# google/uis-rnn

Measured on NVIDIA H100. Metric: predict_frames_per_sec_beam10_256d, higher is better.
Workload: dtype f32

## Files before the change

### uisrnn_b200/csrc/uis_beam.cuh

```cuda
#pragma once
#include "uis_common.cuh"
#include "uis_beam_tc.cuh"
#include "uis_beam_stat.cuh"

namespace uis {

constexpr int kStages = 2;
constexpr int kStageBytes = 48 * 1024;
constexpr int kInitSlot = 0;
#ifndef UIS_CP_BEAM
#define UIS_CP_BEAM 20
#endif
constexpr int kCPBeam = UIS_CP_BEAM;
template <int H> struct BeamCP { static constexpr int value = H > 512 ? 8 : kCPBeam; };
template <int H> __host__ __device__ constexpr int beam_cp() { return BeamCP<H>::value; }
constexpr int kCPCluster = 12;
constexpr int kXchVals = 24;
constexpr int kCPTree = 16;
template <int H> struct TreeCP { static constexpr int value = H > 512 ? 8 : kCPTree; };
template <int H> __host__ __device__ constexpr int tree_cp() { return TreeCP<H>::value; }
constexpr int kMaxLanes = 8;
constexpr int kMaxBeam = 128;
constexpr int kMaxDepth = 4;

// ... 375 lines not shown
  const uint32_t base = smem_u32(mine + tid);
  float sum[NV];
#pragma unroll
  for (int i = 0; i < NV; ++i) sum[i] = 0.f;
  for (unsigned r = 0; r < x.size; ++r) {
    if (r == x.rank) {
#pragma unroll
      for (int i = 0; i < NV; ++i) sum[i] = (r == 0) ? v[i] : __fadd_rn(sum[i], v[i]);
    } else {
      const uint32_t ra = dsmem_addr(base, r);
      float4 t[NV / 4];
#pragma unroll
      for (int i = 0; i < NV / 4; ++i) t[i] = dsmem_ld_f32x4(ra + (uint32_t)(i * NT) * 16u);
#pragma unroll
      for (int i = 0; i < NV / 4; ++i) {
        sum[4 * i + 0] = (r == 0) ? t[i].x : __fadd_rn(sum[4 * i + 0], t[i].x);
        sum[4 * i + 1] = (r == 0) ? t[i].y : __fadd_rn(sum[4 * i + 1], t[i].y);
        sum[4 * i + 2] = (r == 0) ? t[i].z : __fadd_rn(sum[4 * i + 2], t[i].z);
        sum[4 * i + 3] = (r == 0) ? t[i].w : __fadd_rn(sum[4 * i + 3], t[i].w);
      }
    }
  }
#pragma unroll
  for (int i = 0; i < NV; ++i) v[i] = sum[i];
  x.count += 1;
}
template <int NT>
__device__ __forceinline__ void xch_barrier(XchCtx& x, int tid) {
  const unsigned b = x.count & 1u, parity = (x.count >> 1) & 1u;
  named_bar_sync(1, NT);
  if (tid == 0)
    for (unsigned r = 0; r < x.size; ++r)
      if (r != x.rank) mbar_arrive_remote(dsmem_addr(smem_u32(&x.bar[b]), r));
  mbar_wait_cluster(&x.bar[b], parity);
  x.count += 1;
}

struct ColCtx {
  const int* lane;
  const int* src;
  const int* dst;
  const int* vis;
  const long long* girow;
};

template <class C, int NC, bool DEEP, bool XCL = false>
__device__ __forceinline__ void run_pass(const BeamParams& p, const float* ring, uint64_t* full, uint64_t* empty,
                                         unsigned& it, float* XA, float* XB,
                                         const ColCtx cc, int m0, int Mp, float* pool_mean_cta,
                                         float* pool_hidden_cta, const float (&bh)[C::RG], const float (&b1r)[C::UPT],
                                         float b2r, int tid, int lane, long long* ph, long long& tmark,
                                         XchCtx* xc = nullptr) {
  const int xrank = XCL ? (int)xc->rank : 0, xsize = XCL ? (int)xc->size : 1;
  constexpr int H = C::H, D = C::D, NT = C::NT, UPT = C::UPT;
  const int DH = p.depth * H;
  const size_t lane_pool_h = (size_t)p.P * DH, lane_pool_m = (size_t)p.P * D;
  {
    float acc[C::RG][4 * NC];
    lin_pass<C, 3 * H, C::KT_HH, 1, C::RG, NC, true, XCL>(ring, full, empty, it, XA, acc, tid, lane, xrank, xsize);
    if constexpr (XCL) {
      static_assert(!DEEP && 4 * C::RG <= kXchVals, "cluster mode: depth 1");
#pragma unroll
      for (int c = 0; c < NC; ++c) {
        float v[4 * C::RG];
#pragma unroll
        for (int i = 0; i < C::RG; ++i)
#pragma unroll
          for (int q = 0; q < 4; ++q) v[4 * i + q] = acc[i][4 * c + q];
        xch_allreduce<NT, 4 * C::RG>(*xc, v, tid);
#pragma unroll
        for (int i = 0; i < C::RG; ++i)
#pragma unroll
          for (int q = 0; q < 4; ++q) acc[i][4 * c + q] = v[4 * i + q];
      }
    }
#pragma unroll
    for (int u = 0; u < UPT; ++u) {
      const int j = tid + NT * u;
#pragma unroll
      for (int c = 0; c < NC; ++c) {
        const float4 hold = reinterpret_cast<const float4*>(XA + (size_t)j * C::CP)[c];
        const float ho[4] = {hold.x, hold.y, hold.z, hold.w};
        float hn[4];
#pragma unroll
        for (int q = 0; q < 4; ++q) {
          const int m = 4 * c + q;
          hn[q] = 0.f;
          if (m < Mp) {
            const float* gi = p.gi + (size_t)cc.girow[m0 + m] * 3 * H;
            const float r = sigmoid_f32(__fadd_rn(gi[j], __fadd_rn(acc[0 * UPT + u][m], bh[0 * UPT + u])));
            const float z = sigmoid_f32(__fadd_rn(gi[H + j], __fadd_rn(acc[1 * UPT + u][m], bh[1 * UPT + u])));
            const float n = tanhf(__fadd_rn(gi[2 * H + j], __fmul_rn(r, __fadd_rn(acc[2 * UPT + u][m], bh[2 * UPT + u]))));
            hn[q] = __fadd_rn(__fmul_rn(__fsub_rn(ho[q], n), z), n);
            pool_hidden_cta[(size_t)cc.lane[m0 + m] * lane_pool_h + (size_t)cc.dst[m0 + m] * DH + j] = hn[q];
          }
        }
        reinterpret_cast<float4*>(XB + (size_t)j * C::CP)[c] = make_float4(hn[0], hn[1], hn[2], hn[3]);
      }
    }
  }
  if constexpr (DEEP)
  for (int l = 1; l < p.depth; ++l) {
    named_bar_sync(1, NT);
    float acc[C::RG][4 * NC];
    lin_pass<C, 3 * H, C::KT_HH, 1, C::RG, NC>(ring, full, empty, it, XB, acc, tid, lane);
    float ni[UPT][4 * NC];
#pragma unroll
    for (int u = 0; u < UPT; ++u)
#pragma unroll
      for (int m = 0; m < 4 * NC; ++m) { ni[u][m] = acc[2 * UPT + u][m]; acc[2 * UPT + u][m] = 0.f; }
    named_bar_sync(1, NT);
#pragma unroll
    for (int u = 0; u < UPT; ++u) {
      const int j = tid + NT * u;
#pragma unroll
      for (int c = 0; c < NC; ++c) {
        float hv[4];
#pragma unroll
        for (int q = 0; q < 4; ++q) {
          const int m = 4 * c + q;
          hv[q] = (m < Mp) ? pool_hidden_cta[(size_t)cc.lane[m0 + m] * lane_pool_h + (size_t)cc.src[m0 + m] * DH +
                                             (size_t)l * H + j]
                           : 0.f;
        }
        reinterpret_cast<float4*>(XA + (size_t)j * C::CP)[c] = make_float4(hv[0], hv[1], hv[2], hv[3]);
      }
    }
    named_bar_sync(1, NT);
    lin_pass<C, 3 * H, C::KT_HH, 1, C::RG, NC, false>(ring, full, empty, it, XA, acc, tid, lane);
    const float* bi = p.bih_up + (size_t)(l - 1) * 3 * H;
    const float* bhl = p.bhh_up + (size_t)(l - 1) * 3 * H;
    float hn_out[UPT][4 * NC];
#pragma unroll
    for (int u = 0; u < UPT; ++u) {
      const int j = tid + NT * u;
      const float bir = bi[j], biz = bi[H + j], bin = bi[2 * H + j];
      const float bhr = bhl[j], bhz = bhl[H + j], bhn = bhl[2 * H + j];
#pragma unroll
      for (int c = 0; c < NC; ++c) {
        const float4 hold = reinterpret_cast<const float4*>(XA + (size_t)j * C::CP)[c];
        const float ho[4] = {hold.x, hold.y, hold.z, hold.w};
#pragma unroll
        for (int q = 0; q < 4; ++q) {
          const int m = 4 * c + q;
          const float r = sigmoid_f32(__fadd_rn(__fadd_rn(acc[0 * UPT + u][m], bir), bhr));
          const float z = sigmoid_f32(__fadd_rn(__fadd_rn(acc[1 * UPT + u][m], biz), bhz));
          const float n = tanhf(__fadd_rn(__fadd_rn(ni[u][m], bin), __fmul_rn(r, __fadd_rn(acc[2 * UPT + u][m], bhn))));
          const float hnew = __fadd_rn(__fmul_rn(__fsub_rn(ho[q], n), z), n);
          hn_out[u][m] = (m < Mp) ? hnew : 0.f;
          if (m < Mp)
            pool_hidden_cta[(size_t)cc.lane[m0 + m] * lane_pool_h + (size_t)cc.dst[m0 + m] * DH + (size_t)l * H + j] = hnew;
        }
      }
    }
    named_bar_sync(1, NT);
#pragma unroll
    for (int u = 0; u < UPT; ++u)
#pragma unroll
      for (int c = 0; c < NC; ++c)
        reinterpret_cast<float4*>(XB + (size_t)(tid + NT * u) * C::CP)[c] =
            make_float4(hn_out[u][4 * c], hn_out[u][4 * c + 1], hn_out[u][4 * c + 2], hn_out[u][4 * c + 3]);
  }
  named_bar_sync(1, NT);
  if (tid == 0) { const long long now_ = clock64(); ph[2] += now_ - tmark; tmark = now_; }
  {
    float acc[C::R1][4 * NC];
    lin_pass<C, H, C::KT_1, C::KG1, C::R1, NC, true, XCL>(ring, full, empty, it, XB, acc, tid, lane, xrank, xsize);
    float out[UPT][4 * NC];
    ksplit_reduce<C, H, C::KG1, C::R1, UPT, NC>(acc, XA, out, tid);
    if constexpr (XCL) {
      static_assert(UPT * 4 * NC <= kXchVals, "cluster mode: W1 exchange in one round");
      float v[UPT * 4 * NC];
#pragma unroll
      for (int u = 0; u < UPT; ++u)
#pragma unroll
        for (int m = 0; m < 4 * NC; ++m) v[u * 4 * NC + m] = out[u][m];
      xch_allreduce<NT, UPT * 4 * NC>(*xc, v, tid);
#pragma unroll
      for (int u = 0; u < UPT; ++u)
#pragma unroll
        for (int m = 0; m < 4 * NC; ++m) out[u][m] = v[u * 4 * NC + m];
    }
#pragma unroll
    for (int u = 0; u < UPT; ++u)
#pragma unroll
      for (int c = 0; c < NC; ++c) {
        float4 v;
        v.x = fmaxf(__fadd_rn(out[u][4 * c + 0], b1r[u]), 0.f); v.y = fmaxf(__fadd_rn(out[u][4 * c + 1], b1r[u]), 0.f);
        v.z = fmaxf(__fadd_rn(out[u][4 * c + 2], b1r[u]), 0.f); v.w = fmaxf(__fadd_rn(out[u][4 * c + 3], b1r[u]), 0.f);
        reinterpret_cast<float4*>(XA + (size_t)(tid + NT * u) * C::CP)[c] = v;
      }
  }
  named_bar_sync(1, NT);
  if (tid == 0) { const long long now_ = clock64(); ph[3] += now_ - tmark; tmark = now_; }
  {
    float mu_old[4 * NC];
#pragma unroll
    for (int m = 0; m < 4 * NC; ++m)
      mu_old[m] = (m < Mp && tid < D)
                      ? pool_mean_cta[(size_t)cc.lane[m0 + m] * lane_pool_m + (size_t)cc.src[m0 + m] * D + tid]
                      : 0.f;
    float acc[C::R2][4 * NC];
    lin_pass<C, D, C::KT_2, C::KG2, C::R2, NC, true, XCL>(ring, full, empty, it, XA, acc, tid, lane, xrank, xsize);
    float out[1][4 * NC];
    ksplit_reduce<C, D, C::KG2, C::R2, 1, NC>(acc, XA, out, tid);
    if constexpr (XCL) xch_allreduce<NT, 4 * NC>(*xc, out[0], tid);
    if (tid < D) {
#pragma unroll
      for (int m = 0; m < 4 * NC; ++m) {
        if (m < Mp) {
          const float mval = __fadd_rn(out[0][m], b2r);
          const int n = cc.vis[m0 + m];
          const float mu = (n == 0) ? mval
                                    : __fdiv_rn(__fadd_rn(__fmul_rn(mu_old[m], (float)(n - 1)), mval), (float)n);
          pool_mean_cta[(size_t)cc.lane[m0 + m] * lane_pool_m + (size_t)cc.dst[m0 + m] * D + tid] = mu;
        }
      }
    }
  }
}

template <class C, bool DEEP, bool XCL = false>
__device__ __forceinline__ void run_pass_any(const BeamParams& p, const float* ring, uint64_t* full, uint64_t* empty,
                                             unsigned& it, float* XA, float* XB, const ColCtx cc, int m0, int Mp,
                                             float* pool_mean_cta, float* pool_hidden_cta, const float (&bh)[C::RG],
                                             const float (&b1r)[C::UPT], float b2r, int tid, int lane, long long* ph,
                                             long long& tmark, XchCtx* xc = nullptr) {
  const int nc = (Mp + 3) / 4;
#define UIS_RP(NCV, DEEPV) \
  run_pass<C, NCV, DEEPV, XCL>(p, ring, full, empty, it, XA, XB, cc, m0, Mp, pool_mean_cta, pool_hidden_cta, bh, b1r, b2r, tid, lane, ph, tmark, xc)
  if (nc == 1) UIS_RP(1, DEEP); else if (nc == 2) UIS_RP(2, DEEP); else if (nc == 3 || C::CP < 16) UIS_RP(3, DEEP);
  else if (nc == 4 || C::CP < 20) { if constexpr (C::CP >= 16) UIS_RP(4, DEEP); }
  else { if constexpr (C::CP >= 20) UIS_RP(5, DEEP); }
#undef UIS_RP
}

template <int H, int D, int CP, int NT>
__device__ __forceinline__ void stat_pass(const BeamParams& p, const float* sW, float* XA, float* XB, const ColCtx cc, int m0,
                                          int Mp, float* pool_mean_g, float* pool_hidden_g, float* scratch_g, unsigned* bar,
                                          unsigned& epoch, int q, int tid, long long* ph, long long& tmark) {
  using S = StatCfg<H, D>;
  const size_t lane_pool_h = (size_t)p.P * H, lane_pool_m = (size_t)p.P * D;
  stat_dot<H, S::R0, CP, NT>(sW, S::LD, 0, XA, XB, Mp, tid);
  named_bar_sync(1, NT);
  if (tid < S::UG * CP) {
    const int m = tid % CP, u = tid / CP, j = q * S::UG + u;
    if (m < Mp) {
      const float ar = stat_sum<S::R0, CP, NT>(XB, 0 * S::UG + u, m);
      const float az = stat_sum<S::R0, CP, NT>(XB, 1 * S::UG + u, m);
      const float an = stat_sum<S::R0, CP, NT>(XB, 2 * S::UG + u, m);
      const float* gi = p.gi + (size_t)cc.girow[m0 + m] * 3 * H;
      const float r = sigmoid_f32(__fadd_rn(gi[j], __fadd_rn(ar, __ldg(p.bhh + j))));
      const float z = sigmoid_f32(__fadd_rn(gi[H + j], __fadd_rn(az, __ldg(p.bhh + H + j))));
      const float n = tanhf(__fadd_rn(gi[2 * H + j], __fmul_rn(r, __fadd_rn(an, __ldg(p.bhh + 2 * H + j)))));
      const float ho = XA[(size_t)j * CP + m];
      pool_hidden_g[(size_t)cc.lane[m0 + m] * lane_pool_h + (size_t)cc.dst[m0 + m] * H + j] =
          __fadd_rn(__fmul_rn(__fsub_rn(ho, n), z), n);
    }
  }
  stat_group_sync<NT>(bar, epoch, tid);
  if (tid == 0) { const long long now_ = clock64(); ph[2] += now_ - tmark; tmark = now_; }
  for (int i = tid; i < Mp * H; i += NT) {
    const int m = i / H, k = i % H;
    XA[(size_t)k * CP + m] = __ldcg(pool_hidden_g + (size_t)cc.lane[m0 + m] * lane_pool_h + (size_t)cc.dst[m0 + m] * H + k);
  }
  named_bar_sync(1, NT);
  stat_dot<H, S::R1, CP, NT>(sW, S::LD, S::R0, XA, XB, Mp, tid);
  named_bar_sync(1, NT);
  if (tid < S::R1 * CP) {
    const int m = tid % CP, u = tid / CP, j = q * S::R1 + u;
    if (m < Mp)
      scratch_g[(size_t)m * H + j] = fmaxf(__fadd_rn(stat_sum<S::R1, CP, NT>(XB, u, m), __ldg(p.b1 + j)), 0.f);
  }
  stat_group_sync<NT>(bar, epoch, tid);
  if (tid == 0) { const long long now_ = clock64(); ph[3] += now_ - tmark; tmark = now_; }
  for (int i = tid; i < Mp * H; i += NT) {
    const int m = i / H, k = i % H;
    XA[(size_t)k * CP + m] = __ldcg(scratch_g + (size_t)m * H + k);
  }
  named_bar_sync(1, NT);
  stat_dot<H, S::R2, CP, NT>(sW, S::LD, S::R0 + S::R1, XA, XB, Mp, tid);
  named_bar_sync(1, NT);
  if (tid < S::R2 * CP) {
    const int m = tid % CP, u = tid / CP, d = q * S::R2 + u;
    if (m < Mp) {
      const float mval = __fadd_rn(stat_sum<S::R2, CP, NT>(XB, u, m), __ldg(p.b2 + d));
      const int n = cc.vis[m0 + m];
      const float mu_old = __ldcg(pool_mean_g + (size_t)cc.lane[m0 + m] * lane_pool_m + (size_t)cc.src[m0 + m] * D + d);
      const float mu = (n == 0) ? mval : __fdiv_rn(__fadd_rn(__fmul_rn(mu_old, (float)(n - 1)), mval), (float)n);
      pool_mean_g[(size_t)cc.lane[m0 + m] * lane_pool_m + (size_t)cc.dst[m0 + m] * D + d] = mu;
    }
  }
  stat_group_sync<NT>(bar, epoch, tid);
}

template <int H, int D, int N, class Idle>
__device__ __forceinline__ void tc_run_pass(const BeamParams& p, const unsigned char* ring, unsigned char* bop,
                                            const TcBars& tb, unsigned& tbox, const ColCtx cc, int m0, int Mp,
                                            float* pool_mean_cta, float* pool_hidden_cta, float* scratch_cta, int tid,
                                            int lane, int warp, long long* ph, long long& tmark, long long* tstat,
                                            Idle idle_work) {
  using TC = TcCfg<H, D, N>;
  constexpr int NT = 256, NI = N / 8;
  constexpr int KB = (NI == 6) ? 2 : 4, WB = (NI == 6) ? 3 : NI;
  auto hslot = [&](int g, int s) { return pool_hidden_cta + (size_t)(g * p.P + s) * H; };
  auto mslot = [&](int g, int s) { return pool_mean_cta + (size_t)(g * p.P + s) * D; };
  const int wg = warp >> 2;
  const int r0 = wg * 64 + (warp & 3) * 16 + (lane >> 2);
  const int cq = 2 * (lane & 3);
  long long* ts = (tid == 0) ? tstat : nullptr;
  const long long t_in = clock64();
  float acc[TC::NACC];
  auto stage_b = [&](auto src, float scale) {
    const long long w0 = clock64();
    tc_gather_b<H, N, NT>(bop, src, Mp, scale, tid);
    tc_publish_b<NT>();
    if (ts) ts[2] += clock64() - w0;
  };
  if (tid < Mp && (tid == 0 || cc.lane[m0 + tid] != cc.lane[m0 + tid - 1]))
    prefetch_l2_bulk(p.gi + (size_t)cc.girow[m0 + tid] * 3 * H, 3 * H * 4);
  stage_b([&](int m) -> const float* {
    return hslot(cc.lane[m0 + m], cc.src[m0 + m]); }, p.tc_sh);
  if (tid == 0) { const long long now_ = clock64(); ph[1] += now_ - tmark; tmark = now_; }
  idle_work();
  if (tid == 0) { const long long now_ = clock64(); ph[7] += now_ - tmark; tmark = now_; }
  static_assert(H >= NT, "gate parking: 2 * (N / 2) * NT floats within the [N][H] scratch");
  float* park = scratch_cta + tid;
  for (int ut = 0; ut < TC::UT; ++ut) {
    const int j0 = ut * 128 + r0;
    {
      float v[TC::NV];
#pragma unroll
      for (int g = 0; g < 2; ++g) {
        tc_tile<TC>(acc, ring, bop, tb, tbox, wg, lane, ts);
        tc_fold<TC>(acc, v, p.tc_inv_hh);
        const float bh[2] = {__ldg(p.bhh + g * H + j0), __ldg(p.bhh + g * H + j0 + 8)};
#pragma unroll
        for (int q = 0; q < TC::NV; ++q) park[(g * TC::NV + q) * NT] = __fadd_rn(v[q], bh[(q >> 1) & 1]);
      }
    }
    tc_tile<TC>(acc, ring, bop, tb, tbox, wg, lane, ts);
    float an[TC::NV];
    tc_fold<TC>(acc, an, p.tc_inv_hh);
    {
      const float bh[2] = {__ldg(p.bhh + 2 * H + j0), __ldg(p.bhh + 2 * H + j0 + 8)};
#pragma unroll
      for (int q = 0; q < TC::NV; ++q) an[q] = __fadd_rn(an[q], bh[(q >> 1) & 1]);
    }
#pragma unroll
    for (int k0 = 0; k0 < 2 * NI; k0 += KB) {
      float gr[KB][2], gz[KB][2], gn[KB][2], pr[KB][2], pz[KB][2], ho[KB][2];
#pragma unroll
      for (int b = 0; b < KB; ++b) {
        const int i = (k0 + b) >> 1, e = (k0 + b) & 1, m = 8 * i + cq + e;
        if (m < Mp) {
          const float* gi = p.gi + (size_t)cc.girow[m0 + m] * 3 * H + j0;
          const float* hs = hslot(cc.lane[m0 + m], cc.src[m0 + m]) + j0;
#pragma unroll
          for (int h = 0; h < 2; ++h) {
            const int v = 4 * i + 2 * h + e;
            gr[b][h] = __ldg(gi + 8 * h); gz[b][h] = __ldg(gi + H + 8 * h); gn[b][h] = __ldg(gi + 2 * H + 8 * h);
            pr[b][h] = park[v * NT]; pz[b][h] = park[(TC::NV + v) * NT];
            ho[b][h] = hs[8 * h];
          }
        }
      }
#pragma unroll
      for (int b = 0; b < KB; ++b) {
        const int i = (k0 + b) >> 1, e = (k0 + b) & 1, m = 8 * i + cq + e;
        if (m < Mp) {
          float* hd = hslot(cc.lane[m0 + m], cc.dst[m0 + m]) + j0;
#pragma unroll
          for (int h = 0; h < 2; ++h) {
            const int v = 4 * i + 2 * h + e;
            const float rg = sigmoid_f32(__fadd_rn(gr[b][h], pr[b][h]));
            const float zg = sigmoid_f32(__fadd_rn(gz[b][h], pz[b][h]));
            const float ng = tanhf(__fadd_rn(gn[b][h], __fmul_rn(rg, an[v])));
            hd[8 * h] = __fadd_rn(__fmul_rn(__fsub_rn(ho[b][h], ng), zg), ng);
          }
        }
      }
    }
  }
  named_bar_sync(1, NT);
  if (tid == 0) { const long long now_ = clock64(); ph[2] += now_ - tmark; tmark = now_; }
  stage_b([&](int m) -> const float* {
    return hslot(cc.lane[m0 + m], cc.dst[m0 + m]); }, p.tc_sh);
  for (int mt = 0; mt < TC::T2; ++mt) {
    float v1[TC::NV];
    tc_tile<TC>(acc, ring, bop, tb, tbox, wg, lane, ts);
    tc_fold<TC>(acc, v1, p.tc_inv_1);
#pragma unroll
    for (int h = 0; h < 2; ++h) {
      const int j = mt * 128 + r0 + 8 * h;
      const float b1j = __ldg(p.b1 + j);
#pragma unroll
      for (int i = 0; i < NI; ++i)
#pragma unroll
        for (int e = 0; e < 2; ++e) {
          const int m = 8 * i + cq + e;
          if (m < Mp) scratch_cta[(size_t)m * H + j] = fmaxf(__fadd_rn(v1[4 * i + 2 * h + e], b1j), 0.f);
        }
    }
  }
  named_bar_sync(1, NT);
  if (tid == 0) { const long long now_ = clock64(); ph[3] += now_ - tmark; tmark = now_; }
  stage_b([&](int m) -> const float* { return scratch_cta + (size_t)m * H; }, p.tc_sa);
  for (int mt = 0; mt < TC::T3; ++mt) {
    float v2[TC::NV];
    tc_tile<TC>(acc, ring, bop, tb, tbox, wg, lane, ts);
    tc_fold<TC>(acc, v2, p.tc_inv_2);
#pragma unroll
    for (int h = 0; h < 2; ++h) {
      const int d = mt * 128 + r0 + 8 * h;
      const float b2d = __ldg(p.b2 + d);
#pragma unroll
      for (int i0 = 0; i0 < NI; i0 += WB) {
        float mu_old[WB][2];
#pragma unroll
        for (int b = 0; b < WB; ++b)
#pragma unroll
          for (int e = 0; e < 2; ++e) {
            const int m = 8 * (i0 + b) + cq + e;
            if (m < Mp) mu_old[b][e] = mslot(cc.lane[m0 + m], cc.src[m0 + m])[d];
          }
#pragma unroll
        for (int b = 0; b < WB; ++b)
#pragma unroll
          for (int e = 0; e < 2; ++e) {
            const int m = 8 * (i0 + b) + cq + e;
            if (m < Mp) {
              const float mval = __fadd_rn(v2[4 * (i0 + b) + 2 * h + e], b2d);
              const int n = cc.vis[m0 + m];
              const float mu = (n == 0) ? mval : __fdiv_rn(__fadd_rn(__fmul_rn(mu_old[b][e], (float)(n - 1)), mval), (float)n);
              mslot(cc.lane[m0 + m], cc.dst[m0 + m])[d] = mu;
            }
          }
      }
    }
  }
  if (ts) ts[3] += clock64() - t_in;
}

template <int H, int D, bool DEEP, int XM = 0, int TCN = 0>
__global__ void __launch_bounds__(Cfg<H, D>::BLOCK, 1) uis_beam_kernel(const __grid_constant__ BeamParams p) {
  constexpr bool XCL = XM == 1, STAT = XM == 2;
  using C = Cfg<H, D, (XCL || STAT) ? kCPCluster : BeamCP<H>::value>;
  constexpr int NT = C::NT, NW = C::NW, UPT = C::UPT;
  constexpr bool TC = TCN > 0;
  static_assert(!TC || (!DEEP && !XCL && !STAT && NT == 256 && C::REBALANCE), "tensor-core pass: depth 1, one CTA per lane group");
  static_assert(!STAT || (!DEEP && NT == 256), "stationary-weights mode: depth 1, 256 consumer threads");
  using TCC = TcCfg<TC ? H : 512, TC ? D : 256, TC ? TCN : 48>;
  extern __shared__ __align__(128) unsigned char smem_raw[];
  unsigned char* smem = TC ? reinterpret_cast<unsigned char*>((reinterpret_cast<uintptr_t>(smem_raw) + 1023) & ~(uintptr_t)1023)
                           : smem_raw;
  const int B = p.B, Kcap = p.Kcap, G = p.G;
  const SmemLayout L_ = make_layout<H, D, C::CP, XCL, TCN, STAT>(B, Kcap, G);
  const SmemLayout& L = TC ? p.tc_layout : L_;
  if constexpr (TC)
    if (p.tc_layout.total == 0) __trap();
  const int sq = STAT ? (int)(blockIdx.x % kStatGroup) : 0, sgroup = STAT ? (int)(blockIdx.x / kStatGroup) : 0;
  float* ring = reinterpret_cast<float*>(smem + L.ring);
  float* XA = reinterpret_cast<float*>(smem + L.xa);
  float* XB = reinterpret_cast<float*>(smem + L.xb);
  float* wv = reinterpret_cast<float*>(smem + L.wv);
  int* colarr = reinterpret_cast<int*>(smem + L.cols);
  uint64_t* full = reinterpret_cast<uint64_t*>(smem + L.bars);
  uint64_t* empty = full + (TC ? TCC::STAGES : kStages);
  volatile int* misc = reinterpret_cast<volatile int*>(smem + L.misc);
  TcBars tb{full, empty};

  const int tid = threadIdx.x, lane = tid & 31, warp = tid >> 5;

  if (tid == 0) {
    if constexpr (TC) {
      for (int s = 0; s < TCC::STAGES; ++s) {
        mbar_init(&tb.full[s], 1);
        mbar_init(&tb.empty[s], NW);
      }
    } else {
      for (int s = 0; s < kStages; ++s) {
        mbar_init(&full[s], 1);
        mbar_init(&empty[s], NW);
      }
    }
    for (int i = 0; i < 16; ++i) misc[i] = 0;
    if constexpr (TC)
      for (int i = 16; i < 20; ++i) reinterpret_cast<long long*>(smem + L.phase)[i] = 0;
    if constexpr (XCL) {
      uint64_t* xbar = reinterpret_cast<uint64_t*>(smem + L.xbar);
      mbar_init(&xbar[0], cluster_nctarank() - 1);
      mbar_init(&xbar[1], cluster_nctarank() - 1);
      misc[MI_QNEXT] = (int)cluster_id_x();
    }
    if constexpr (STAT) misc[MI_QNEXT] = sgroup;
    fence_mbar_init();
  }
  __syncthreads();
  if constexpr (XCL) cluster_sync_all();

  if (warp >= NW) {
    if constexpr (STAT) return;
    if constexpr (TC) asm volatile("setmaxnreg.dec.sync.aligned.u32 40;");
    else if constexpr (C::REBALANCE) asm volatile("setmaxnreg.dec.sync.aligned.u32 24;");
    if constexpr (TC) {
      if (warp == NW) tc_producer_loop<TCC, H>(&p.tc_wmap, reinterpret_cast<unsigned char*>(ring), tb, &misc[MI_DONE]);
    } else {
      if (warp == NW && lane == 0) producer_loop<C, XCL>(p, ring, full, empty, misc);
    }
    return;
  }
  if constexpr (TC) asm volatile("setmaxnreg.inc.sync.aligned.u32 232;");
  else if constexpr (C::REBALANCE && !STAT) asm volatile("setmaxnreg.inc.sync.aligned.u32 240;");

  auto lane_base = [&](int g) -> unsigned char* { return smem + L.lanes + (size_t)g * L.lane_stride; };
  auto LSp = [&](int g) -> volatile int* { return reinterpret_cast<volatile int*>(lane_base(g) + L.l_ls); };
  const int DH = p.depth * H;
  const size_t pool_m_stride = (size_t)p.P * D, pool_h_stride = (size_t)p.P * DH;
  float* pool_mean_cta = p.pool_mean + (size_t)(STAT ? sgroup : blockIdx.x) * G * pool_m_stride;
  float* pool_hidden_cta = p.pool_hidden + (size_t)(STAT ? sgroup : blockIdx.x) * G * pool_h_stride;
  unsigned* bp_cta = p.bp + (size_t)blockIdx.x * G * p.maxN * B;
  const unsigned PW = (unsigned)(p.P + 31) / 32;
  const float INF = __int_as_float(0x7f800000);
  const int bbits = B > 32 ? 7 : 5;

  float bh[C::RG], b1r[UPT];
#pragma unroll
  for (int i = 0; i < C::RG; ++i) bh[i] = TC ? 0.f : p.bhh[(i / UPT) * H + tid + NT * (i % UPT)];
#pragma unroll
  for (int u = 0; u < UPT; ++u) b1r[u] = TC ? 0.f : p.b1[tid + NT * u];
  const float b2r = (tid < D && !TC) ? p.b2[tid] : 0.f;
  unsigned tc_boxes = 0;
  float* tc_scratch_cta = TC ? p.tc_scratch + (size_t)blockIdx.x * (TC ? TCN : 1) * H : nullptr;
  if (tid < D) wv[tid] = p.wvec[tid];
  unsigned stat_epoch = 0;
  if constexpr (STAT) stat_load_weights<H, D, NT>(ring, p.whh_t, p.w1_t, p.w2_t, sq, tid);
  for (int g = 0; g < G; ++g) {
    if (tid < D) pool_mean_cta[g * pool_m_stride + (size_t)kInitSlot * D + tid] = p.mean0[tid];
    for (int q = tid; q < DH; q += NT) pool_hidden_cta[g * pool_h_stride + (size_t)kInitSlot * DH + q] = p.hidden0[q];
  }

  int* collane = colarr; int* colsrc = colarr + G * B; int* colnew = colarr + 2 * G * B;
  int* colvis = colarr + 3 * G * B;
  long long* colrow = reinterpret_cast<long long*>(colarr + 4 * G * B);
  const ColCtx cc{collane, colsrc, colnew, colvis, colrow};
  XchCtx xc{reinterpret_cast<float*>(smem + L.xch), reinterpret_cast<uint64_t*>(smem + L.xbar),
            XCL ? cluster_ctarank() : 0u, XCL ? cluster_nctarank() : 1u, 0u};
  const int xsize = (int)xc.size;
  const bool tap_leader = (!XCL || xc.rank == 0) && (!STAT || sq == 0);

  unsigned it = 0;
  long long* ph = reinterpret_cast<long long*>(smem + L.phase);
  if (tid == 0) {
    for (int i = 0; i < 16; ++i) ph[i] = 0;
    ph[10] = clock64();
  }
  long long& tmark = ph[10];
  long long& st_cols = ph[11]; long long& st_pass = ph[12]; long long& st_cand = ph[13]; long long& st_steps = ph[14];
  long long& st_maxk = ph[15];
#define UIS_PHASE(i)                         \
  do {                                       \
    if (tid == 0) {                          \
      const long long now_ = clock64();      \
      ph[i] += now_ - tmark;                 \
      tmark = now_;                          \
    }                                        \
  } while (0)

  auto lane_fetch = [&](int g) {
    volatile int* ls = LSp(g);
    for (;;) {
      int uidx;
      if constexpr (XCL) {
        uidx = misc[MI_QNEXT];
        misc[MI_QNEXT] = uidx + (int)cluster_nclusters_x();
      } else if constexpr (STAT) {
        uidx = misc[MI_QNEXT];
        misc[MI_QNEXT] = uidx + (int)(gridDim.x / kStatGroup);
      } else {
        uidx = atomicAdd(p.queue, 1);
      }
      if (uidx >= p.U) { ls[LS_ACTIVE] = 0; ls[LS_FRESH] = 0; return; }
      const int u = p.order[uidx];
      const long long row0 = p.row_off[u];
      const int N = (int)(p.row_off[u + 1] - row0);
      if (N == 0) {
        p.status[u] = 0;
        if (p.spk_out) p.spk_out[u] = 0;
        if (p.nbest_count) p.nbest_count[u] = 0;
        for (int j = 0; j < p.n_best; ++j) nbest_store(p, u, j, -1, nullptr, nullptr);
        if (p.dbg_final_scores && tap_leader) {
          for (int b = 0; b < B; ++b) p.dbg_final_scores[(size_t)u * B + b] = INF;
          if (p.dbg_final_k) p.dbg_final_k[u] = 0;
        }
        continue;
      }
      ls[LS_U] = u; ls[LS_N] = N; ls[LS_TN] = p.T * N; ls[LS_T] = 0; ls[LS_NB] = 1; ls[LS_GEN] = 0;
      ls[LS_ACTIVE] = 1; ls[LS_FAILED] = 0; ls[LS_TRACED] = (u == p.trace_utt) && tap_leader; ls[LS_ERR] = 0;
      ls[LS_ROW0_LO] = (int)(row0 & 0xffffffffll); ls[LS_ROW0_HI] = (int)(row0 >> 32);
      ls[LS_DBGROWS_LO] = 0; ls[LS_DBGROWS_HI] = 0; ls[LS_FRESH] = 1;
      ls[LS_KHI] = spk_max(p, u); ls[LS_KLO] = spk_min(p, u);
      for (unsigned w = 0; w < PW; ++w) reinterpret_cast<unsigned*>(lane_base(g) + L.l_scored)[w] = 0;
      int* meta = reinterpret_cast<int*>(lane_base(g) + L.l_meta);
      meta[0] = 0; meta[B] = -1; meta[2 * B] = 0; reinterpret_cast<float*>(meta)[3 * B] = 0.f;
      if (u == p.trace_utt && tap_leader && p.dbg_off) p.dbg_off[0] = 0;
      return;
    }
  };
  if (G > NW) __trap();
  auto team_of = [&]() { return warp / (NW / G); };
  auto team_sync = [&]() {
    const int TW = NW / G;
    if (TW == 1) __syncwarp();
    else named_bar_sync(2 + warp / TW, TW * 32);
  };

  auto lane_prefetch = [&](int g, int t, int ttid, int TT) {
    volatile int* ls = LSp(g);
    const long long row0 = ((long long)ls[LS_ROW0_HI] << 32) | (unsigned)ls[LS_ROW0_LO];
    const long long r = row0 + (t % ls[LS_N]);
    float* xts = reinterpret_cast<float*>(lane_base(g) + L.l_xt) + (t & 1) * D;
    for (int q = ttid; q < D / 4; q += TT) cp_async16(xts + q * 4, p.x + (size_t)r * D + q * 4);
  };

  float* pool_mse_cta = p.pool_mse + (size_t)blockIdx.x * G * p.P;
  constexpr int kSlotList = 64;
  auto score_lane_slots = [&](int g, bool next, int ttid, int twarp, int TW) {
    unsigned* used = reinterpret_cast<unsigned*>(lane_base(g) + L.l_used);
    unsigned* scored = reinterpret_cast<unsigned*>(lane_base(g) + L.l_scored);
    unsigned* slist = reinterpret_cast<unsigned*>(smem + L.slist) + kSlotList * g;
    volatile int* ls = LSp(g);
    const float* xs = reinterpret_cast<const float*>(lane_base(g) + L.l_xt) + ((ls[LS_T] + (next ? 1 : 0)) & 1) * D;
    const float* mu_g = pool_mean_cta + g * pool_m_stride;
    float* mse_g = pool_mse_cta + (size_t)g * p.P;
    for (;;) {
      if (twarp == 0) {
        int ntot = 0;
        for (int w0 = 0; w0 < (int)PW; w0 += 32) {
          const int w = w0 + lane;
          unsigned bits = 0;
          if (w < (int)PW) bits = next ? (scored[w] & ~used[w]) : (used[w] & ~scored[w]);
          const int n = __popc(bits);
          int incl = n;
#pragma unroll
          for (int o = 1; o < 32; o <<= 1) {
            const int v = __shfl_up_sync(0xffffffffu, incl, o);
            if (lane >= o) incl += v;
          }
          int pos = ntot + incl - n;
          unsigned done = 0;
          while (bits && pos < kSlotList) {
            const int bit = __ffs(bits) - 1;
            bits &= bits - 1;
            done |= 1u << bit;
            slist[pos++] = (unsigned)(w * 32 + bit);
          }
          if (done) { if (next) used[w] |= done; else scored[w] |= done; }
          ntot += __shfl_sync(0xffffffffu, incl, 31);
        }
        if (lane == 0) ls[LS_NLIST] = ntot;
      }
      team_sync();
      const int ntot = ls[LS_NLIST], nlist = min(ntot, kSlotList);
      constexpr int kBatch = 4;
      for (int f0 = twarp * kBatch; f0 < nlist; f0 += TW * kBatch) {
        int cslot[kBatch];
        float4 m4[kBatch][(D + 127) / 128];
#pragma unroll
        for (int q = 0; q < kBatch; ++q) {
          const int f = f0 + q;
          cslot[q] = -1;
          if (f < nlist) {
            cslot[q] = (int)slist[f];
            const float* mu = mu_g + (size_t)cslot[q] * D;
#pragma unroll
            for (int i = 0; i < (D + 127) / 128; ++i)
              if (lane * 4 + i * 128 < D)
                m4[q][i] = STAT ? __ldcg(reinterpret_cast<const float4*>(mu + lane * 4 + i * 128))
                                : *reinterpret_cast<const float4*>(mu + lane * 4 + i * 128);
          }
        }
        float acc[kBatch], d0sq[kBatch];
#pragma unroll
        for (int q = 0; q < kBatch; ++q) {
          acc[q] = 0.f; d0sq[q] = 1.f;
#pragma unroll
          for (int i = 0; i < (D + 127) / 128; ++i) {
            const int d = lane * 4 + i * 128;
            if (d < D && cslot[q] >= 0) {
              const float4 x4 = *reinterpret_cast<const float4*>(xs + d);
              const float4 w4 = *reinterpret_cast<const float4*>(wv + d);
              const float e0 = __fsub_rn(m4[q][i].x, x4.x), e1 = __fsub_rn(m4[q][i].y, x4.y);
              const float e2 = __fsub_rn(m4[q][i].z, x4.z), e3 = __fsub_rn(m4[q][i].w, x4.w);
              const float q0 = __fmul_rn(e0, e0);
              if (d == 0) d0sq[q] = q0;
              acc[q] = __fadd_rn(acc[q], __fmul_rn(q0, w4.x));
              acc[q] = __fadd_rn(acc[q], __fmul_rn(__fmul_rn(e1, e1), w4.y));
              acc[q] = __fadd_rn(acc[q], __fmul_rn(__fmul_rn(e2, e2), w4.z));
              acc[q] = __fadd_rn(acc[q], __fmul_rn(__fmul_rn(e3, e3), w4.w));
            }
          }
        }
#pragma unroll
        for (int o = 16; o > 0; o >>= 1) {
#pragma unroll
          for (int q = 0; q < kBatch; ++q) acc[q] = __fadd_rn(acc[q], __shfl_xor_sync(0xffffffffu, acc[q], o));
        }
        float my_acc = acc[0], my_d0 = __shfl_sync(0xffffffffu, d0sq[0], 0);
        int my_slot = cslot[0];
#pragma unroll
        for (int q = 1; q < kBatch; ++q) {
          const float dq = __shfl_sync(0xffffffffu, d0sq[q], 0);
          if (lane == q) { my_acc = acc[q]; my_d0 = dq; my_slot = cslot[q]; }
        }
        if (lane < kBatch && my_slot >= 0) {
          if (my_d0 == 0.f) my_acc = __fdiv_rn(my_acc, 0.f);
          mse_g[my_slot] = my_acc;
        }
      }
      team_sync();
      if (ntot <= kSlotList) break;
    }
  };

  if (team_of() < G) {
    const int g = team_of(), TT = (NW / G) * 32, ttid = tid - g * TT;
    if (ttid == 0) lane_fetch(g);
    team_sync();
    if (LSp(g)[LS_ACTIVE]) lane_prefetch(g, 0, ttid, TT);
    cp_async_commit();
  }
  named_bar_sync(1, NT);

  for (;;) {
    if (team_of() < G) {
      const int g = team_of(), TW = NW / G, TT = TW * 32, ttid = tid - g * TT, twarp = warp - g * TW;
      volatile int* ls = LSp(g);
      unsigned char* lb = lane_base(g);
      const bool active = ls[LS_ACTIVE] != 0;
      const int gen = ls[LS_GEN], t = ls[LS_T];
      const int* mK = reinterpret_cast<const int*>(lb + L.l_meta) + gen * 4 * B;
      const int* mLast = mK + B; const int* mTot = mK + 2 * B;
// ... 432 lines not shown
```

Baseline: 2.237 million.

## Keep GRU gates in registers and prefetch operands ahead of tensor-core tiles

The GRU update pass no longer parks the r/z pre-activations in shared scratch. The r and z gates are now computed straight into registers, and the input-gate rows and biases are loaded before the tensor-core tiles, so their latency overlaps the MMA work. The mean-update pass likewise prefetches the old means, visit counts and biases before its tile, and the b1 bias load is hoisted ahead of the tile. This removes the shared-memory round trips and exposed global-load latency, at the cost of more live registers per thread and possible spills.

```diff
diff --git a/uisrnn_b200/csrc/uis_beam.cuh b/uisrnn_b200/csrc/uis_beam.cuh
--- a/uisrnn_b200/csrc/uis_beam.cuh
+++ b/uisrnn_b200/csrc/uis_beam.cuh
@@ -701,7 +701,6 @@
                                             Idle idle_work) {
   using TC = TcCfg<H, D, N>;
   constexpr int NT = 256, NI = N / 8;
-  constexpr int KB = (NI == 6) ? 2 : 4, WB = (NI == 6) ? 3 : NI;
   auto hslot = [&](int g, int s) { return pool_hidden_cta + (size_t)(g * p.P + s) * H; };
   auto mslot = [&](int g, int s) { return pool_mean_cta + (size_t)(g * p.P + s) * D; };
   const int wg = warp >> 2;
@@ -723,76 +722,82 @@
   if (tid == 0) { const long long now_ = clock64(); ph[1] += now_ - tmark; tmark = now_; }
   idle_work();
   if (tid == 0) { const long long now_ = clock64(); ph[7] += now_ - tmark; tmark = now_; }
-  static_assert(H >= NT, "gate parking: 2 * (N / 2) * NT floats within the [N][H] scratch");
-  float* park = scratch_cta + tid;
   for (int ut = 0; ut < TC::UT; ++ut) {
     const int j0 = ut * 128 + r0;
-    {
+    float gi3[3][TC::NV] = {}, rz[2][TC::NV] = {}, ho[TC::NV] = {}, bh[3][2];
+    auto load_gi = [&](int g) {
+#pragma unroll
+      for (int i = 0; i < NI; ++i)
+#pragma unroll
+        for (int e = 0; e < 2; ++e) {
+          const int m = 8 * i + cq + e;
+          if (m < Mp) {
+            const float* gi = p.gi + (size_t)cc.girow[m0 + m] * 3 * H + g * H + j0;
+#pragma unroll
+            for (int h = 0; h < 2; ++h) gi3[g][4 * i + 2 * h + e] = __ldg(gi + 8 * h);
+          }
+        }
+    };
+    auto load_bias = [&](int g) {
+#pragma unroll
+      for (int h = 0; h < 2; ++h) bh[g][h] = __ldg(p.bhh + g * H + j0 + 8 * h);
+    };
+    load_gi(0); load_bias(0);
+    load_gi(1); load_bias(1);
+#pragma unroll
+    for (int g = 0; g < 2; ++g) {
       float v[TC::NV];
-#pragma unroll
-      for (int g = 0; g < 2; ++g) {
-        tc_tile<TC>(acc, ring, bop, tb, tbox, wg, lane, ts);
-        tc_fold<TC>(acc, v, p.tc_inv_hh);
-        const float bh[2] = {__ldg(p.bhh + g * H + j0), __ldg(p.bhh + g * H + j0 + 8)};
-#pragma unroll
-        for (int q = 0; q < TC::NV; ++q) park[(g * TC::NV + q) * NT] = __fadd_rn(v[q], bh[(q >> 1) & 1]);
-      }
-    }
+      tc_tile<TC>(acc, ring, bop, tb, tbox, wg, lane, ts);
+      tc_fold<TC>(acc, v, p.tc_inv_hh);
+#pragma unroll
+      for (int q = 0; q < TC::NV; ++q)
+        if (8 * (q >> 2) + cq + (q & 1) < Mp) rz[g][q] = sigmoid_f32(__fadd_rn(gi3[g][q], __fadd_rn(v[q], bh[g][(q >> 1) & 1])));
+    }
+    load_gi(2);
     tc_tile<TC>(acc, ring, bop, tb, tbox, wg, lane, ts);
     float an[TC::NV];
     tc_fold<TC>(acc, an, p.tc_inv_hh);
-    {
-      const float bh[2] = {__ldg(p.bhh + 2 * H + j0), __ldg(p.bhh + 2 * H + j0 + 8)};
-#pragma unroll
-      for (int q = 0; q < TC::NV; ++q) an[q] = __fadd_rn(an[q], bh[(q >> 1) & 1]);
-    }
-#pragma unroll
-    for (int k0 = 0; k0 < 2 * NI; k0 += KB) {
-      float gr[KB][2], gz[KB][2], gn[KB][2], pr[KB][2], pz[KB][2], ho[KB][2];
-#pragma unroll
-      for (int b = 0; b < KB; ++b) {
-        const int i = (k0 + b) >> 1, e = (k0 + b) & 1, m = 8 * i + cq + e;
+    load_bias(2);
+#pragma unroll
+    for (int i = 0; i < NI; ++i)
+#pragma unroll
+      for (int e = 0; e < 2; ++e) {
+        const int m = 8 * i + cq + e;
         if (m < Mp) {
-          const float* gi = p.gi + (size_t)cc.girow[m0 + m] * 3 * H + j0;
           const float* hs = hslot(cc.lane[m0 + m], cc.src[m0 + m]) + j0;
+#pragma unroll
+          for (int h = 0; h < 2; ++h) ho[4 * i + 2 * h + e] = hs[8 * h];
+        }
+      }
+#pragma unroll
+    for (int i = 0; i < NI; ++i)
+#pragma unroll
+      for (int e = 0; e < 2; ++e) {
+        const int m = 8 * i + cq + e;
+        if (m < Mp) {
+          float* hd = hslot(cc.lane[m0 + m], cc.dst[m0 + m]) + j0;
 #pragma unroll
           for (int h = 0; h < 2; ++h) {
             const int v = 4 * i + 2 * h + e;
-            gr[b][h] = __ldg(gi + 8 * h); gz[b][h] = __ldg(gi + H + 8 * h); gn[b][h] = __ldg(gi + 2 * H + 8 * h);
-            pr[b][h] = park[v * NT]; pz[b][h] = park[(TC::NV + v) * NT];
-            ho[b][h] = hs[8 * h];
-          }
-        }
-      }
-#pragma unroll
-      for (int b = 0; b < KB; ++b) {
-        const int i = (k0 + b) >> 1, e = (k0 + b) & 1, m = 8 * i + cq + e;
-        if (m < Mp) {
-          float* hd = hslot(cc.lane[m0 + m], cc.dst[m0 + m]) + j0;
-#pragma unroll
-          for (int h = 0; h < 2; ++h) {
-            const int v = 4 * i + 2 * h + e;
-            const float rg = sigmoid_f32(__fadd_rn(gr[b][h], pr[b][h]));
-            const float zg = sigmoid_f32(__fadd_rn(gz[b][h], pz[b][h]));
-            const float ng = tanhf(__fadd_rn(gn[b][h], __fmul_rn(rg, an[v])));
-            hd[8 * h] = __fadd_rn(__fmul_rn(__fsub_rn(ho[b][h], ng), zg), ng);
-          }
-        }
-      }
-    }
+            const float ng = tanhf(__fadd_rn(gi3[2][v], __fmul_rn(rz[0][v], __fadd_rn(an[v], bh[2][h]))));
+            hd[8 * h] = __fadd_rn(__fmul_rn(__fsub_rn(ho[v], ng), rz[1][v]), ng);
+          }
+        }
+      }
   }
   named_bar_sync(1, NT);
   if (tid == 0) { const long long now_ = clock64(); ph[2] += now_ - tmark; tmark = now_; }
   stage_b([&](int m) -> const float* {
     return hslot(cc.lane[m0 + m], cc.dst[m0 + m]); }, p.tc_sh);
   for (int mt = 0; mt < TC::T2; ++mt) {
+    const float b1r[2] = {__ldg(p.b1 + mt * 128 + r0), __ldg(p.b1 + mt * 128 + r0 + 8)};
     float v1[TC::NV];
     tc_tile<TC>(acc, ring, bop, tb, tbox, wg, lane, ts);
     tc_fold<TC>(acc, v1, p.tc_inv_1);
 #pragma unroll
     for (int h = 0; h < 2; ++h) {
       const int j = mt * 128 + r0 + 8 * h;
-      const float b1j = __ldg(p.b1 + j);
+      const float b1j = b1r[h];
 #pragma unroll
       for (int i = 0; i < NI; ++i)
 #pragma unroll
@@ -806,37 +811,42 @@
   if (tid == 0) { const long long now_ = clock64(); ph[3] += now_ - tmark; tmark = now_; }
   stage_b([&](int m) -> const float* { return scratch_cta + (size_t)m * H; }, p.tc_sa);
   for (int mt = 0; mt < TC::T3; ++mt) {
+    const int d0 = mt * 128 + r0;
+    const float b2r[2] = {__ldg(p.b2 + d0), __ldg(p.b2 + d0 + 8)};
+    float mu_old[TC::NV] = {};
+    int vis[2 * NI] = {};
+#pragma unroll
+    for (int i = 0; i < NI; ++i)
+#pragma unroll
+      for (int e = 0; e < 2; ++e) {
+        const int m = 8 * i + cq + e;
+        if (m < Mp) {
+          vis[2 * i + e] = cc.vis[m0 + m];
+          const float* ms = mslot(cc.lane[m0 + m], cc.src[m0 + m]) + d0;
+#pragma unroll
+          for (int h = 0; h < 2; ++h) mu_old[4 * i + 2 * h + e] = ms[8 * h];
+        }
+      }
     float v2[TC::NV];
     tc_tile<TC>(acc, ring, bop, tb, tbox, wg, lane, ts);
     tc_fold<TC>(acc, v2, p.tc_inv_2);
 #pragma unroll
-    for (int h = 0; h < 2; ++h) {
-      const int d = mt * 128 + r0 + 8 * h;
-      const float b2d = __ldg(p.b2 + d);
-#pragma unroll
-      for (int i0 = 0; i0 < NI; i0 += WB) {
-        float mu_old[WB][2];
-#pragma unroll
-        for (int b = 0; b < WB; ++b)
-#pragma unroll
-          for (int e = 0; e < 2; ++e) {
-            const int m = 8 * (i0 + b) + cq + e;
-            if (m < Mp) mu_old[b][e] = mslot(cc.lane[m0 + m], cc.src[m0 + m])[d];
-          }
-#pragma unroll
-        for (int b = 0; b < WB; ++b)
-#pragma unroll
-          for (int e = 0; e < 2; ++e) {
-            const int m = 8 * (i0 + b) + cq + e;
-            if (m < Mp) {
-              const float mval = __fadd_rn(v2[4 * (i0 + b) + 2 * h + e], b2d);
-              const int n = cc.vis[m0 + m];
-              const float mu = (n == 0) ? mval : __fdiv_rn(__fadd_rn(__fmul_rn(mu_old[b][e], (float)(n - 1)), mval), (float)n);
-              mslot(cc.lane[m0 + m], cc.dst[m0 + m])[d] = mu;
-            }
-          }
-      }
-    }
+    for (int i = 0; i < NI; ++i)
+#pragma unroll
+      for (int e = 0; e < 2; ++e) {
+        const int m = 8 * i + cq + e;
+        if (m < Mp) {
+          const int n = vis[2 * i + e];
+          float* md = mslot(cc.lane[m0 + m], cc.dst[m0 + m]) + d0;
+#pragma unroll
+          for (int h = 0; h < 2; ++h) {
+            const int v = 4 * i + 2 * h + e;
+            const float mval = __fadd_rn(v2[v], b2r[h]);
+            const float mu = (n == 0) ? mval : __fdiv_rn(__fadd_rn(__fmul_rn(mu_old[v], (float)(n - 1)), mval), (float)n);
+            md[8 * h] = mu;
+          }
+        }
+      }
   }
   if (ts) ts[3] += clock64() - t_in;
 }
```

Measured after the change: 2.306 million (median of 6 runs). 3.1% higher.
